# zhoujiahuan1991/ICCV2025-UPP

Hardware: AMD Instinct MI355X
Metric: point-clouds/sec fwd+bwd, UPP/Point-MAE N=1024 G=64 k=32 (higher is better)
Workload: dtype f32

## Files before the change

iccv2025-upp_amd/upp_hip/csrc/adapter.hip:

```cpp
#include "common.h"

namespace {

typedef float f32x16 __attribute__((ext_vector_type(16)));
constexpr int kH = 32;
constexpr int kRows = 32;
constexpr int kLG = 33;
constexpr int kAW = 8;
constexpr int kAT = 64 * kAW;

__device__ __forceinline__ int trow(int r, int lk) { return (r & 3) + 8 * (r >> 2) + 4 * lk; }
__device__ __forceinline__ void zero16(f32x16 &a) {
#pragma unroll
    for (int r = 0; r < 16; ++r) a[r] = 0.0f;
}
__device__ __forceinline__ float gelu_f(float x) { return 0.5f * x * (1.0f + erff(x * 0.70710678118654752440f)); }
__device__ __forceinline__ float gelu_grad(float x) {
    const float cdf = 0.5f * (1.0f + erff(x * 0.70710678118654752440f));
    const float pdf = 0.39894228040143267794f * expf(-0.5f * x * x);
    return cdf + x * pdf;
}

template <int NK, typename FA, typename FB>
__device__ __forceinline__ void mfma_chain(f32x16 &acc, FA fa, FB fb) {
// ... 308 lines not shown
#pragma unroll
    for (int t = 0; t < 2; ++t)
#pragma unroll
        for (int i = 0; i < NI; ++i)
            w1v[t][i] = *reinterpret_cast<const float4 *>(a.W1 + (size_t)(16 * t + r) * D + wave * KW + 16 * i + 4 * g);
#pragma unroll
    for (int t = 0; t < NT; ++t)
#pragma unroll
        for (int i = 0; i < 2; ++i)
            w2v[t][i] = *reinterpret_cast<const float4 *>(a.W2 + (size_t)(16 * (wave * NT + t) + r) * kH + 16 * i + 4 * g);

    {
        float gv[E], bv[E], ybv[E];
#pragma unroll
        for (int e = 0; e < E; ++e) {
            gv[e] = a.gamma[lane + 64 * e];
            bv[e] = a.beta[lane + 64 * e];
            ybv[e] = a.ybias ? a.ybias[lane + 64 * e] : 0.0f;
        }
        float xv[RW][E], yv[RW][E];
        int rowi[RW], bi[RW];
        [[maybe_unused]] int ci[RW];
        [[maybe_unused]] float pa[RW][E];
#pragma unroll
        for (int q = 0; q < RW; ++q) {
            const int row = min(row0 + wave * RW + q, R - 1);
            const int b = row / a.Lout, t = row - b * a.Lout;
            const int src = a.mode == 3 ? (t == 0 ? 0 : t + a.P) : (a.mode == 4 ? t + a.P : t);
            const size_t off = ((size_t)b * a.Lin + src) * D;
            rowi[q] = row; bi[q] = b;
            if constexpr (PROP) ci[q] = src - (a.Lin - a.T);
#pragma unroll
            for (int e = 0; e < E; ++e) {
                xv[q][e] = a.x[off + lane + 64 * e];
                yv[q][e] = a.y ? a.y[off + lane + 64 * e] : 0.0f;
            }
            for (int pp = 1; pp < a.yparts; ++pp) {
                float yp[E];
#pragma unroll
                for (int e = 0; e < E; ++e) yp[e] = a.y[(size_t)pp * a.ystride + off + lane + 64 * e];
#pragma unroll
                for (int e = 0; e < E; ++e) yv[q][e] += yp[e];
            }
        }
        if constexpr (PROP) {
            constexpr int kNb = 8, EC = 3;
            static_assert(E % EC == 0, "shape");
            float mu[E], rs[E], ga[E], be[E];
#pragma unroll
            for (int e = 0; e < E; ++e) {
                mu[e] = a.bn_mean[lane + 64 * e]; rs[e] = a.bn_rstd[lane + 64 * e];
                ga[e] = a.bn_gamma[lane + 64 * e]; be[e] = a.bn_beta[lane + 64 * e];
            }
#pragma unroll
            for (int q = 0; q < RW; ++q) {
                float acc[E];
#pragma unroll
                for (int e = 0; e < E; ++e) acc[e] = 0.0f;
                if (ci[q] >= 0) {
                    int j[kNb], cr[kNb];
                    float w[kNb], scr[kNb];
                    const size_t tok = ((size_t)bi[q] * a.T + ci[q]) * kNb;
#pragma unroll
                    for (int k = 0; k < kNb; ++k) { j[k] = a.idx8[tok + k]; w[k] = a.w8[tok + k]; }
#pragma unroll
                    for (int k = 0; k < kNb; ++k) cr[k] = a.i2[bi[q] * a.G2 + j[k]];
#pragma unroll
                    for (int k = 0; k < kNb; ++k) scr[k] = a.u ? floorf(a.keep + a.u[cr[k] / a.Lin]) / a.keep : 1.0f;
#pragma unroll
                    for (int h = 0; h < E; h += EC) {
                        float lv[EC][kNb], cx[EC][kNb], cy[EC][kNb];
#pragma unroll
                        for (int e = 0; e < EC; ++e)
#pragma unroll
                            for (int k = 0; k < kNb; ++k) {
                                const int c = lane + 64 * (h + e);
                                lv[e][k] = a.pooled[((size_t)bi[q] * a.G2 + j[k]) * D + c];
                                cx[e][k] = a.x[(size_t)cr[k] * D + c];
                                cy[e][k] = a.y[(size_t)cr[k] * D + c];
                            }
#pragma unroll
                        for (int e = 0; e < EC; ++e)
#pragma unroll
                            for (int k = 0; k < kNb; ++k) {
                                const float cv = __builtin_fmaf(cy[e][k] + ybv[h + e], scr[k], cx[e][k]);
                                const float lcv = ((lv[e][k] - mu[h + e]) * rs[h + e]) * ga[h + e] + be[h + e];
                                acc[h + e] += (lcv + 0.3f * cv) * w[k];
                            }
                    }
                }
#pragma unroll
                for (int e = 0; e < E; ++e) pa[q][e] = ci[q] >= 0 ? 0.3f * acc[e] : 0.0f;
            }
        }
#pragma unroll
        for (int q = 0; q < RW; ++q) {
            const int rr = wave * RW + q;
            const bool live = row0 + rr < R;
            const float sc = a.y ? (a.u ? floorf(a.keep + a.u[bi[q]]) / a.keep : 1.0f) : 0.0f;
            float v[E];
            float s = 0.0f;
#pragma unroll
            for (int e = 0; e < E; ++e) {
                float val = xv[q][e];
                if (a.y) val = __builtin_fmaf(yv[q][e] + ybv[e], sc, val);
                if constexpr (PROP) val = val + pa[q][e];
                v[e] = val;
                s += val;
            }
            const float mean = wave_sum_f32(s) / (float)D;
            float qq = 0.0f;
#pragma unroll
            for (int e = 0; e < E; ++e) { const float dv = v[e] - mean; qq = __builtin_fmaf(dv, dv, qq); }
            const float rstd = 1.0f / sqrtf(wave_sum_f32(qq) / (float)D + a.eps);
#pragma unroll
            for (int e = 0; e < E; ++e) {
                const float h = __builtin_fmaf((v[e] - mean) * rstd, gv[e], bv[e]);
                Hs[rr * LDH + lane + 64 * e] = live ? h : 0.0f;
                Vs[rr * LDH + lane + 64 * e] = v[e];
                if (live) a.xo[(size_t)rowi[q] * D + lane + 64 * e] = v[e];
            }
// ... 564 lines not shown
```

iccv2025-upp_amd/upp_hip/csrc/prop.hip:

```cpp
#include "common.h"

int upp_bn_finalize_launch(const float *part, int slabs, int per, int rows, int C, int training, float momentum, float eps,
                           float *running_mean, float *running_var, float *mean, float *rstd, hipStream_t st);

namespace {

constexpr int kMaxE = 8;
constexpr int kNb = 8;

__global__ __launch_bounds__(256) void prop_pool_fwd_kernel(const float *__restrict__ X, const int32_t *__restrict__ i1,
                                                            const float *__restrict__ u, float keep, float *__restrict__ pooled,
                                                            uint8_t *__restrict__ amax, int groups, int D) {
    const int lane = threadIdx.x & 63;
    const int g = blockIdx.x * 4 + __builtin_amdgcn_readfirstlane(threadIdx.x >> 6);
    if (g >= groups) return;
    const float f = 1.0f + (u ? floorf(keep + u[g]) / keep : 1.0f);
    float mx[kMaxE], sm[kMaxE];
    int am[kMaxE];
#pragma unroll
    for (int e = 0; e < kMaxE; ++e) { mx[e] = -__builtin_inff(); sm[e] = 0.0f; am[e] = 0; }
    int rows8[kNb];
#pragma unroll
    for (int k = 0; k < kNb; ++k) rows8[k] = i1[g * kNb + k];
    float val[kNb][kMaxE];
#pragma unroll
    for (int k = 0; k < kNb; ++k)
#pragma unroll
        for (int e = 0; e < kMaxE; ++e) val[k][e] = X[(size_t)rows8[k] * D + min(lane + 64 * e, D - 1)];
#pragma unroll
    for (int k = 0; k < kNb; ++k)
#pragma unroll
        for (int e = 0; e < kMaxE; ++e) {
            const float v = val[k][e] * f;
            if (v > mx[e]) { mx[e] = v; am[e] = k; }
            sm[e] += v;
        }
#pragma unroll
    for (int e = 0; e < kMaxE; ++e) {
        const int c = lane + 64 * e;
        if (c < D) { pooled[(size_t)g * D + c] = mx[e] + sm[e] * 0.125f; amax[(size_t)g * D + c] = (uint8_t)am[e]; }
    }
}

__device__ __forceinline__ int collect_hits(const int32_t *list, int n, int key, int *hits, int cap, int lane, int &q0) {
    int cnt = 0;
    int q = q0;
    for (; q < n && cnt + 64 <= cap; q += 64) {
        const int me = q + lane;
        const bool pred = me < n && list[me] == key;
        const unsigned long long mask = __ballot(pred);
        if (mask) {
            const int pos = cnt + __popcll(mask & ((1ull << lane) - 1ull));
            if (pred) hits[pos] = me;
            cnt += __popcll(mask);
        }
    }
    q0 = q;
    __builtin_amdgcn_wave_barrier();
    return cnt;
}
// ... 314 lines not shown
    }
}

__global__ __launch_bounds__(256) void prop_interp_bn_fwd_kernel(const float *__restrict__ X, const float *__restrict__ pooled,
                                                                 const float *__restrict__ mean, const float *__restrict__ rstd,
                                                                 const float *__restrict__ gamma, const float *__restrict__ beta,
                                                                 const int32_t *__restrict__ i2, const int32_t *__restrict__ idx8,
                                                                 const float *__restrict__ w8, float *__restrict__ out, int B, int Lp,
                                                                 int T, int G2, int D) {
    const int wgx = xcd_contiguous((int)blockIdx.x, (int)gridDim.x);
    const int lane = threadIdx.x & 63;
    const int r = wgx * 4 + __builtin_amdgcn_readfirstlane(threadIdx.x >> 6);
    if (r >= B * Lp) return;
    const int b = r / Lp, t = r - b * Lp;
    const int i = t - (Lp - T);
    int cc[kMaxE];
    float xv[kMaxE], acc[kMaxE];
#pragma unroll
    for (int e = 0; e < kMaxE; ++e) { cc[e] = min(lane + 64 * e, D - 1); xv[e] = X[(size_t)r * D + cc[e]]; acc[e] = 0.0f; }
    if (i >= 0) {
        int j[kNb], cr[kNb];
        float w[kNb];
#pragma unroll
        for (int k = 0; k < kNb; ++k) { j[k] = idx8[((size_t)b * T + i) * kNb + k]; w[k] = w8[((size_t)b * T + i) * kNb + k]; }
        float mu[kMaxE], rs[kMaxE], ga[kMaxE], be[kMaxE];
#pragma unroll
        for (int e = 0; e < kMaxE; ++e) { mu[e] = mean[cc[e]]; rs[e] = rstd[cc[e]]; ga[e] = gamma[cc[e]]; be[e] = beta[cc[e]]; }
#pragma unroll
        for (int k = 0; k < kNb; ++k) cr[k] = i2[b * G2 + j[k]];
#pragma unroll
        for (int h = 0; h < kMaxE; h += 4) {
            float lv[4][kNb], cv[4][kNb];
#pragma unroll
            for (int e = 0; e < 4; ++e)
#pragma unroll
                for (int k = 0; k < kNb; ++k) { lv[e][k] = pooled[((size_t)b * G2 + j[k]) * D + cc[h + e]]; cv[e][k] = X[(size_t)cr[k] * D + cc[h + e]]; }
#pragma unroll
            for (int e = 0; e < 4; ++e)
#pragma unroll
                for (int k = 0; k < kNb; ++k) {
                    const float lcv = ((lv[e][k] - mu[h + e]) * rs[h + e]) * ga[h + e] + be[h + e];
                    acc[h + e] += (lcv + 0.3f * cv[e][k]) * w[k];
                }
            if (64 * (h + 4) >= D) break;
        }
    }
#pragma unroll
    for (int e = 0; e < kMaxE; ++e) {
        const int c = lane + 64 * e;
        if (c < D) out[(size_t)r * D + c] = xv[e] + (i >= 0 ? 0.3f * acc[e] : 0.0f);
    }
}

__global__ __launch_bounds__(256) void prop_c2_csr_kernel(const float *__restrict__ g_out, const int32_t *__restrict__ start8,
                                                          const int32_t *__restrict__ perm8, const float *__restrict__ w8,
                                                          const float *__restrict__ pooled, const float *__restrict__ mean,
                                                          const float *__restrict__ rstd, float *__restrict__ g_c2,
                                                          float *__restrict__ part, int B, int Lp, int T, int G2, int D) {
    const int wgx = xcd_contiguous((int)blockIdx.x, (int)gridDim.x);
    __shared__ float sh[2][4][64 * kMaxE];
    const int lane = threadIdx.x & 63, wave = __builtin_amdgcn_readfirstlane(threadIdx.x >> 6);
    const int gj = wgx * 4 + wave;
    const int groups = B * G2;
    if (gj < groups) {
        int cc[kMaxE];
        float acc[kMaxE], pv[kMaxE], mu[kMaxE], rs[kMaxE];
#pragma unroll
        for (int e = 0; e < kMaxE; ++e) {
            cc[e] = min(lane + 64 * e, D - 1); acc[e] = 0.0f;
            pv[e] = pooled[(size_t)gj * D + cc[e]]; mu[e] = mean[cc[e]]; rs[e] = rstd[cc[e]];
        }
        const int s = start8[gj], eend = start8[gj + 1];
        for (int h0 = s; h0 < eend; h0 += 8) {
            int q[8];
#pragma unroll
            for (int t = 0; t < 8; ++t) q[t] = perm8[min(h0 + t, eend - 1)];
            float w[8];
            const float *grow[8];
#pragma unroll
            for (int t = 0; t < 8; ++t) {
                const int tok = q[t] / kNb;
                const int bb = tok / T, ii = tok - bb * T;
                w[t] = w8[q[t]];
                grow[t] = g_out + ((size_t)bb * Lp + (Lp - T) + ii) * D;
            }
            float gv[kMaxE][8];
#pragma unroll
            for (int e = 0; e < kMaxE; ++e)
#pragma unroll
                for (int t = 0; t < 8; ++t) gv[e][t] = grow[t][cc[e]];
#pragma unroll
            for (int t = 0; t < 8; ++t) {
                const float wt = h0 + t < eend ? w[t] : 0.0f;
#pragma unroll
                for (int e = 0; e < kMaxE; ++e) acc[e] += gv[e][t] * wt;
            }
        }
#pragma unroll
        for (int e = 0; e < kMaxE; ++e) {
            const int c = lane + 64 * e;
            if (c < D) {
                const float gl = 0.3f * acc[e];
                g_c2[(size_t)gj * D + c] = gl;
                sh[0][wave][c] = gl;
                sh[1][wave][c] = gl * ((pv[e] - mu[e]) * rs[e]);
            }
        }
    }
    __syncthreads();
    const int nw = min(4, groups - (int)wgx * 4);
    for (int c = threadIdx.x; c < D; c += 256) {
        float s0 = 0.0f, s1 = 0.0f;
        for (int w = 0; w < nw; ++w) { s0 += sh[0][w][c]; s1 += sh[1][w][c]; }
        part[((size_t)wgx * 2 + 0) * D + c] = s0;
        part[((size_t)wgx * 2 + 1) * D + c] = s1;
    }
}

__global__ __launch_bounds__(256) void prop_bn_grad_kernel(const float *__restrict__ part, int wgs, int D, float *__restrict__ g_gamma,
                                                           float *__restrict__ g_beta) {
    __shared__ float sb[4][64], sg[4][64];
    const int lane = threadIdx.x & 63, wave = threadIdx.x >> 6;
    const int c = blockIdx.x * 64 + lane;
    const int cc = min(c, D - 1);
    float ab = 0.0f, ag = 0.0f;
    for (int w0 = wave; w0 < wgs; w0 += 4 * 8) {
        float pb[8], pg[8];
#pragma unroll
        for (int t = 0; t < 8; ++t) {
            const int w = min(w0 + 4 * t, wgs - 1);
            pb[t] = part[((size_t)w * 2 + 0) * D + cc]; pg[t] = part[((size_t)w * 2 + 1) * D + cc];
        }
#pragma unroll
        for (int t = 0; t < 8; ++t) if (w0 + 4 * t < wgs) { ab += pb[t]; ag += pg[t]; }
    }
    sb[wave][lane] = ab; sg[wave][lane] = ag;
    __syncthreads();
    if (wave == 0 && c < D) {
        g_beta[c] = (sb[0][lane] + sb[1][lane]) + (sb[2][lane] + sb[3][lane]);
        g_gamma[c] = (sg[0][lane] + sg[1][lane]) + (sg[2][lane] + sg[3][lane]);
    }
}

__global__ __launch_bounds__(256) void prop_x_csr_kernel(const float *__restrict__ g_out, const float *__restrict__ g_c2,
                                                         const float *__restrict__ pooled, const uint8_t *__restrict__ amax,
                                                         const float *__restrict__ mean, const float *__restrict__ rstd,
                                                         const float *__restrict__ gamma, const float *__restrict__ g_gamma,
                                                         const float *__restrict__ g_beta, const float *__restrict__ u, float keep,
                                                         const int32_t *__restrict__ start1, const int32_t *__restrict__ perm1,
                                                         const int32_t *__restrict__ start2, const int32_t *__restrict__ perm2,
                                                         float *__restrict__ g_X, int rows, int groups, int D, int training) {
    const int wgx = xcd_contiguous((int)blockIdx.x, (int)gridDim.x);
    const int lane = threadIdx.x & 63;
    const int r = wgx * 4 + __builtin_amdgcn_readfirstlane(threadIdx.x >> 6);
    if (r >= rows) return;
    const int s1 = start1[r], e1 = start1[r + 1], s2 = start2[r], e2 = start2[r + 1];
    int cc[kMaxE];
    float acc[kMaxE], mu[kMaxE], rs[kMaxE], ga[kMaxE], c1[kMaxE], c2[kMaxE];
    const float inv_n = 1.0f / (float)groups;
#pragma unroll
    for (int e = 0; e < kMaxE; ++e) {
        cc[e] = min(lane + 64 * e, D - 1);
        acc[e] = g_out[(size_t)r * D + cc[e]];
        mu[e] = mean[cc[e]]; rs[e] = rstd[cc[e]]; ga[e] = gamma[cc[e]];
        c1[e] = 0.0f; c2[e] = 0.0f;
    }
    if (training) {
#pragma unroll
        for (int e = 0; e < kMaxE; ++e) { c1[e] = g_beta[cc[e]]; c2[e] = g_gamma[cc[e]]; }
    }
#pragma unroll
    for (int e = 0; e < kMaxE; ++e) { c1[e] *= inv_n; c2[e] *= inv_n; }
    for (int h0 = s2; h0 < e2; h0 += 2) {
        const int m0 = perm2[h0], m1 = perm2[min(h0 + 1, e2 - 1)];
        float a0[kMaxE], a1[kMaxE];
#pragma unroll
        for (int e = 0; e < kMaxE; ++e) { a0[e] = g_c2[(size_t)m0 * D + cc[e]]; a1[e] = g_c2[(size_t)m1 * D + cc[e]]; }
        const float f1 = h0 + 1 < e2 ? 0.3f : 0.0f;
#pragma unroll
        for (int e = 0; e < kMaxE; ++e) { acc[e] += 0.3f * a0[e]; acc[e] += f1 * a1[e]; }
    }
    auto add_entries = [&](int b0, int b1) {
        for (int h0 = b0; h0 < b1; h0 += 4) {
            int g[4], k[4];
            float f[4];
#pragma unroll
            for (int t = 0; t < 4; ++t) { const int q = perm1[min(h0 + t, b1 - 1)]; g[t] = q / kNb; k[t] = q - g[t] * kNb; }
#pragma unroll
            for (int t = 0; t < 4; ++t) f[t] = h0 + t < b1 ? 1.0f + (u ? floorf(keep + u[g[t]]) / keep : 1.0f) : 0.0f;
            float gl[kMaxE][4], pv[kMaxE][4];
            int am[kMaxE][4];
#pragma unroll
            for (int e = 0; e < kMaxE; ++e)
#pragma unroll
                for (int t = 0; t < 4; ++t) {
                    const size_t o = (size_t)g[t] * D + cc[e];
                    gl[e][t] = g_c2[o]; pv[e][t] = pooled[o]; am[e][t] = amax[o];
                }
#pragma unroll
            for (int e = 0; e < kMaxE; ++e)
#pragma unroll
                for (int t = 0; t < 4; ++t) {
                    const float xh = (pv[e][t] - mu[e]) * rs[e];
                    const float gp = (ga[e] * rs[e]) * (training ? gl[e][t] - c1[e] - xh * c2[e] : gl[e][t]);
                    acc[e] += gp * f[t] * (0.125f + (am[e][t] == k[t] ? 1.0f : 0.0f));
                }
        }
    };
    constexpr int kRowChunk = 64;
    if (e1 - s1 <= kRowChunk) {
        add_entries(s1, e1);
    } else {
        float head[kMaxE];
#pragma unroll
        for (int e = 0; e < kMaxE; ++e) head[e] = 0.0f;
        for (int c0 = s1; c0 < e1; c0 += kRowChunk) {
            if (c0 > s1) {
#pragma unroll
                for (int e = 0; e < kMaxE; ++e) { head[e] += acc[e]; acc[e] = 0.0f; }
            }
            add_entries(c0, min(e1, c0 + kRowChunk));
        }
#pragma unroll
        for (int e = 0; e < kMaxE; ++e) acc[e] += head[e];
    }
#pragma unroll
    for (int e = 0; e < kMaxE; ++e) { const int c = lane + 64 * e; if (c < D) g_X[(size_t)r * D + c] = acc[e]; }
}

__device__ __forceinline__ float res_scale(const float *u_dp, float keep_dp, int b) {
    return u_dp ? floorf(keep_dp + u_dp[b]) / keep_dp : 1.0f;
}

__global__ __launch_bounds__(256) void prop_pool_res_stats_kernel(const float *__restrict__ x2, const float *__restrict__ m,
                                                                  const float *__restrict__ mbias, const float *__restrict__ u_dp,
                                                                  float keep_dp, int Lp, const int32_t *__restrict__ i1,
                                                                  const float *__restrict__ u, float keep, float *__restrict__ pooled,
                                                                  uint8_t *__restrict__ amax, float *__restrict__ part, int groups, int D) {
    const int wgx = xcd_contiguous((int)blockIdx.x, (int)gridDim.x);
    __shared__ float sh[4][64 * kMaxE];
    const int lane = threadIdx.x & 63, wave = __builtin_amdgcn_readfirstlane(threadIdx.x >> 6);
    const int g = wgx * 4 + wave;
    if (g < groups) {
        const float f = 1.0f + (u ? floorf(keep + u[g]) / keep : 1.0f);
        int rows8[kNb];
        float sc[kNb];
#pragma unroll
        for (int k = 0; k < kNb; ++k) rows8[k] = i1[g * kNb + k];
#pragma unroll
        for (int k = 0; k < kNb; ++k) sc[k] = res_scale(u_dp, keep_dp, rows8[k] / Lp);
        float xv[kNb][kMaxE], mv[kNb][kMaxE], mb[kMaxE];
#pragma unroll
        for (int k = 0; k < kNb; ++k)
#pragma unroll
            for (int e = 0; e < kMaxE; ++e) {
                const size_t o = (size_t)rows8[k] * D + min(lane + 64 * e, D - 1);
                xv[k][e] = x2[o]; mv[k][e] = m[o];
            }
#pragma unroll
        for (int e = 0; e < kMaxE; ++e) mb[e] = mbias ? mbias[min(lane + 64 * e, D - 1)] : 0.0f;
#pragma unroll
        for (int e = 0; e < kMaxE; ++e) {
            float mx = -__builtin_inff(), sm = 0.0f;
            int am = 0;
#pragma unroll
            for (int k = 0; k < kNb; ++k) {
                const float v = __builtin_fmaf(mv[k][e] + mb[e], sc[k], xv[k][e]) * f;
                if (v > mx) { mx = v; am = k; }
                sm += v;
            }
            const int c = lane + 64 * e;
            const float pv = mx + sm * 0.125f;
            if (c < D) { pooled[(size_t)g * D + c] = pv; amax[(size_t)g * D + c] = (uint8_t)am; sh[wave][c] = pv; }
        }
    }
    __syncthreads();
    const int nw = min(4, groups - (int)wgx * 4);
    for (int c = threadIdx.x; c < D; c += 256) {
        float sum = 0.0f;
        for (int w = 0; w < nw; ++w) sum += sh[w][c];
        const float mean = sum / (float)nw;
        float m2 = 0.0f;
        for (int w = 0; w < nw; ++w) { const float dv = sh[w][c] - mean; m2 = __builtin_fmaf(dv, dv, m2); }
        part[((size_t)wgx * 2 + 0) * D + c] = sum;
        part[((size_t)wgx * 2 + 1) * D + c] = m2;
    }
}

__global__ __launch_bounds__(256) void prop_x_csr_res_kernel(const float *__restrict__ g_out, const float *__restrict__ g_c2,
                                                             const float *__restrict__ pooled, const uint8_t *__restrict__ amax,
                                                             const float *__restrict__ mean, const float *__restrict__ rstd,
                                                             const float *__restrict__ gamma, const float *__restrict__ g_gamma,
                                                             const float *__restrict__ g_beta, const float *__restrict__ u, float keep,
                                                             const int32_t *__restrict__ start1, const int32_t *__restrict__ perm1,
                                                             const int32_t *__restrict__ start2, const int32_t *__restrict__ perm2,
                                                             const float *__restrict__ u_dp, float keep_dp, int Lp,
                                                             float *__restrict__ g_x2, float *__restrict__ g_m, int rows, int groups, int D,
                                                             int training) {
    const int wgx = xcd_contiguous((int)blockIdx.x, (int)gridDim.x);
    const int lane = threadIdx.x & 63;
    const int r = wgx * 4 + __builtin_amdgcn_readfirstlane(threadIdx.x >> 6);
    if (r >= rows) return;
    const int s1 = start1[r], e1 = start1[r + 1], s2 = start2[r], e2 = start2[r + 1];
    const float sc = res_scale(u_dp, keep_dp, r / Lp);
    int cc[kMaxE];
    float acc[kMaxE], mu[kMaxE], rs[kMaxE], ga[kMaxE], c1[kMaxE], c2[kMaxE];
    const float inv_n = 1.0f / (float)groups;
#pragma unroll
    for (int e = 0; e < kMaxE; ++e) {
        cc[e] = min(lane + 64 * e, D - 1);
        acc[e] = g_out[(size_t)r * D + cc[e]];
        mu[e] = mean[cc[e]]; rs[e] = rstd[cc[e]]; ga[e] = gamma[cc[e]];
        c1[e] = 0.0f; c2[e] = 0.0f;
    }
    if (training) {
#pragma unroll
        for (int e = 0; e < kMaxE; ++e) { c1[e] = g_beta[cc[e]]; c2[e] = g_gamma[cc[e]]; }
    }
#pragma unroll
    for (int e = 0; e < kMaxE; ++e) { c1[e] *= inv_n; c2[e] *= inv_n; }
    for (int h0 = s2; h0 < e2; h0 += 2) {
        const int m0 = perm2[h0], m1 = perm2[min(h0 + 1, e2 - 1)];
        float a0[kMaxE], a1[kMaxE];
#pragma unroll
        for (int e = 0; e < kMaxE; ++e) { a0[e] = g_c2[(size_t)m0 * D + cc[e]]; a1[e] = g_c2[(size_t)m1 * D + cc[e]]; }
        const float f1 = h0 + 1 < e2 ? 0.3f : 0.0f;
#pragma unroll
        for (int e = 0; e < kMaxE; ++e) { acc[e] += 0.3f * a0[e]; acc[e] += f1 * a1[e]; }
    }
    auto add_entries = [&](int b0, int b1) {
        for (int h0 = b0; h0 < b1; h0 += 4) {
            int g[4], k[4];
            float f[4];
#pragma unroll
            for (int t = 0; t < 4; ++t) { const int q = perm1[min(h0 + t, b1 - 1)]; g[t] = q / kNb; k[t] = q - g[t] * kNb; }
#pragma unroll
            for (int t = 0; t < 4; ++t) f[t] = h0 + t < b1 ? 1.0f + (u ? floorf(keep + u[g[t]]) / keep : 1.0f) : 0.0f;
            float gl[kMaxE][4], pv[kMaxE][4];
            int am[kMaxE][4];
#pragma unroll
            for (int e = 0; e < kMaxE; ++e)
#pragma unroll
                for (int t = 0; t < 4; ++t) {
                    const size_t o = (size_t)g[t] * D + cc[e];
                    gl[e][t] = g_c2[o]; pv[e][t] = pooled[o]; am[e][t] = amax[o];
                }
#pragma unroll
            for (int e = 0; e < kMaxE; ++e)
#pragma unroll
                for (int t = 0; t < 4; ++t) {
                    const float xh = (pv[e][t] - mu[e]) * rs[e];
                    const float gp = (ga[e] * rs[e]) * (training ? gl[e][t] - c1[e] - xh * c2[e] : gl[e][t]);
                    acc[e] += gp * f[t] * (0.125f + (am[e][t] == k[t] ? 1.0f : 0.0f));
                }
        }
    };
    constexpr int kRowChunk = 64;
    if (e1 - s1 <= kRowChunk) {
        add_entries(s1, e1);
    } else {
        float head[kMaxE];
#pragma unroll
        for (int e = 0; e < kMaxE; ++e) head[e] = 0.0f;
        for (int c0 = s1; c0 < e1; c0 += kRowChunk) {
            if (c0 > s1) {
#pragma unroll
                for (int e = 0; e < kMaxE; ++e) { head[e] += acc[e]; acc[e] = 0.0f; }
            }
            add_entries(c0, min(e1, c0 + kRowChunk));
        }
#pragma unroll
        for (int e = 0; e < kMaxE; ++e) acc[e] += head[e];
    }
#pragma unroll
    for (int e = 0; e < kMaxE; ++e) {
        const int c = lane + 64 * e;
        if (c < D) { g_x2[(size_t)r * D + c] = acc[e]; g_m[(size_t)r * D + c] = acc[e] * sc; }
    }
}

__global__ __launch_bounds__(256) void prop_index_kernel(const float *__restrict__ c1, const float *__restrict__ c2,
                                                         const int64_t *__restrict__ i1, const int64_t *__restrict__ i2, int gather_idx,
                                                         int B, int T, int G2, int Lp, int off, float eps,
                                                         int32_t *__restrict__ i1a, int32_t *__restrict__ i2a,
                                                         int32_t *__restrict__ idx8, float *__restrict__ w8) {
    const int lane = threadIdx.x & 63;
    const int wg = blockIdx.x * 4 + __builtin_amdgcn_readfirstlane(threadIdx.x >> 6);
    {
        const int n1 = B * G2 * kNb, n2 = B * G2;
        const int e = wg * 64 + lane;
        if (e < n1 + n2) {
            const bool first = e < n1;
            const long long v = first ? i1[e] : i2[e - n1];
            long long r;
            if (gather_idx) {
                const int bsmp = first ? e / (G2 * kNb) : (e - n1) / G2;
                r = (long long)bsmp * Lp + off + v;
            } else {
                const int G = Lp - off;
                r = (v / G) * Lp + off + v % G;
            }
            if (first) i1a[e] = (int32_t)r; else i2a[e - n1] = (int32_t)r;
        }
    }
    if (wg >= B * T) return;
    const int b = wg / T;
    const float *a = c1 + (size_t)wg * 3;
    const float ax = a[0], ay = a[1], az = a[2];
    const int j = min(lane, G2 - 1);
    const float *q = c2 + ((size_t)b * G2 + j) * 3;
    const float bx = q[0], by = q[1], bz = q[2];
    float d = -2.0f * __builtin_fmaf(az, bz, __builtin_fmaf(ay, by, ax * bx));
    d += (ax * ax + ay * ay) + az * az;
    d += (bx * bx + by * by) + bz * bz;
    const uint32_t bits = __float_as_uint(d);
    uint32_t img = lane < G2 ? ((bits & 0x80000000u) ? ~bits : (bits | 0x80000000u)) : 0xFFFFFFFFu;
    float dk[kNb];
    int jk[kNb];
#pragma unroll
    for (int k = 0; k < kNb; ++k) {
        const uint32_t m = wave_min_u32(img);
        const int win = __builtin_ctzll(__ballot(img == m));
        jk[k] = win;
        dk[k] = __uint_as_float((m & 0x80000000u) ? (m & 0x7FFFFFFFu) : ~m);
        if (lane == win) img = 0xFFFFFFFFu;
    }
    float rc[kNb], sum = 0.0f;
#pragma unroll
    for (int k = 0; k < kNb; ++k) { rc[k] = 1.0f / (dk[k] + eps); sum += rc[k]; }
    if (lane < kNb) {
        float wv = 0.0f; int jv = 0;
// ... 167 lines not shown
    if (lds > 64 * 1024) return UPP_E_RANGE;
    const size_t lds_perm = lds + (size_t)2 * n * sizeof(int32_t);
    if (lds_perm <= 150 * 1024) {
        static std::atomic<bool> raised{false};
        if (!raised) {
            hipError_t e = hipFuncSetAttribute(reinterpret_cast<const void *>(csr_build_kernel<true>),
                                               hipFuncAttributeMaxDynamicSharedMemorySize, 150 * 1024);
            if (e != hipSuccess) return (int)e;
            raised = true;
        }
        hipLaunchKernelGGL(csr_build_kernel<true>, dim3(1), dim3(kCsrThreads), lds_perm, (hipStream_t)stream, keys, n, seg_len, seg_rows, rows,
                           start, perm);
    } else {
        hipLaunchKernelGGL(csr_build_kernel<false>, dim3(1), dim3(kCsrThreads), lds, (hipStream_t)stream, keys, n, seg_len, seg_rows, rows,
                           start, perm);
    }
    return upp_launch_status();
}

extern "C" long long upp_prop_part_floats(int groups, int D) {
    if (groups < 1 || D < 1) return 0;
    return (long long)((groups + 3) / 4) * 2 * D;
}

extern "C" int upp_prop_fwd(const float *X, const int32_t *i1, const float *u, float keep, const int32_t *i2, const int32_t *idx8,
                            const float *w8, const float *gamma, const float *beta, float *running_mean, float *running_var,
                            float momentum, float eps, int training, float *pooled, uint8_t *amax, float *part, float *mean,
                            float *rstd, float *out, int B, int Lp, int T, int G2, int D, void *stream) {
    if (!X || !i1 || !i2 || !idx8 || !w8 || !gamma || !beta || !pooled || !amax || !part || !mean || !rstd || !out) return UPP_E_BADARG;
    if (B < 1 || Lp < T || T < 1 || G2 < 1 || D < 1) return UPP_E_BADARG;
    if (!training && (!running_mean || !running_var)) return UPP_E_BADARG;
    if (D > 64 * kMaxE) return UPP_E_RANGE;
    hipStream_t st = (hipStream_t)stream;
    const int groups = B * G2, wgs = (groups + 3) / 4;
    hipLaunchKernelGGL(prop_pool_stats_kernel, dim3(wgs), dim3(256), 0, st, X, i1, u, keep, pooled, amax, part, groups, D);
    upp_bn_finalize_launch(part, wgs, 4, groups, D, training, momentum, eps, running_mean, running_var, mean, rstd, st);
    hipLaunchKernelGGL(prop_interp_bn_fwd_kernel, rows_grid((long long)B * Lp), dim3(256), 0, st, X, pooled, mean, rstd, gamma, beta, i2,
                       idx8, w8, out, B, Lp, T, G2, D);
    return upp_launch_status();
}

extern "C" int upp_prop_bwd(const float *g_out, const float *pooled, const uint8_t *amax, const float *mean, const float *rstd,
                            const float *gamma, const float *u, float keep, const float *w8, const int32_t *start1,
                            const int32_t *perm1, const int32_t *start2, const int32_t *perm2, const int32_t *start8,
                            const int32_t *perm8, int training, float *g_c2, float *part, float *g_gamma, float *g_beta, float *g_X,
                            int B, int Lp, int T, int G2, int D, void *stream) {
    if (!g_out || !pooled || !amax || !mean || !rstd || !gamma || !w8 || !start1 || !perm1 || !start2 || !perm2 || !start8 || !perm8 ||
        !g_c2 || !part || !g_gamma || !g_beta || !g_X)
        return UPP_E_BADARG;
    if (B < 1 || Lp < T || T < 1 || G2 < 1 || D < 1) return UPP_E_BADARG;
    if (D > 64 * kMaxE) return UPP_E_RANGE;
    hipStream_t st = (hipStream_t)stream;
    const int groups = B * G2, wgs = (groups + 3) / 4;
    hipLaunchKernelGGL(prop_c2_csr_kernel, dim3(wgs), dim3(256), 0, st, g_out, start8, perm8, w8, pooled, mean, rstd, g_c2, part, B, Lp, T,
                       G2, D);
    hipLaunchKernelGGL(prop_bn_grad_kernel, dim3((D + 63) / 64), dim3(256), 0, st, part, wgs, D, g_gamma, g_beta);
    hipLaunchKernelGGL(prop_x_csr_kernel, rows_grid((long long)B * Lp), dim3(256), 0, st, g_out, g_c2, pooled, amax, mean, rstd, gamma,
                       g_gamma, g_beta, u, keep, start1, perm1, start2, perm2, g_X, B * Lp, groups, D, training);
    return upp_launch_status();
}

extern "C" int upp_prop_res_pool_fwd(const float *x2, const float *m, const float *mbias, const float *u_dp, float keep_dp,
                                     const int32_t *i1, const float *u, float keep, float *running_mean, float *running_var,
                                     float momentum, float eps, int training, float *pooled, uint8_t *amax, float *part, float *mean,
                                     float *rstd, int B, int Lp, int G2, int D, void *stream) {
    if (!x2 || !m || !i1 || !pooled || !amax || !part || !mean || !rstd) return UPP_E_BADARG;
    if (B < 1 || Lp < 1 || G2 < 1 || D < 1 || !(keep_dp > 0.0f) || !(keep > 0.0f)) return UPP_E_BADARG;
    if (!training && (!running_mean || !running_var)) return UPP_E_BADARG;
    if (D > 64 * kMaxE) return UPP_E_RANGE;
    hipStream_t st = (hipStream_t)stream;
    const int groups = B * G2, wgs = (groups + 3) / 4;
    hipLaunchKernelGGL(prop_pool_res_stats_kernel, dim3(wgs), dim3(256), 0, st, x2, m, mbias, u_dp, keep_dp, Lp, i1, u, keep, pooled, amax,
                       part, groups, D);
    upp_bn_finalize_launch(part, wgs, 4, groups, D, training, momentum, eps, running_mean, running_var, mean, rstd, st);
    return upp_launch_status();
}

extern "C" int upp_prop_res_bwd(const float *g_out, const float *pooled, const uint8_t *amax, const float *mean, const float *rstd,
                                const float *gamma, const float *u, float keep, const float *w8, const int32_t *start1,
                                const int32_t *perm1, const int32_t *start2, const int32_t *perm2, const int32_t *start8,
                                const int32_t *perm8, int training, const float *u_dp, float keep_dp, float *g_c2, float *part,
                                float *g_gamma, float *g_beta, float *g_x2, float *g_m, int B, int Lp, int T, int G2, int D, void *stream) {
    if (!g_out || !pooled || !amax || !mean || !rstd || !gamma || !w8 || !start1 || !perm1 || !start2 || !perm2 || !start8 || !perm8 ||
        !g_c2 || !part || !g_gamma || !g_beta || !g_x2 || !g_m)
        return UPP_E_BADARG;
    if (B < 1 || Lp < T || T < 1 || G2 < 1 || D < 1 || !(keep_dp > 0.0f)) return UPP_E_BADARG;
    if (D > 64 * kMaxE) return UPP_E_RANGE;
    hipStream_t st = (hipStream_t)stream;
    const int groups = B * G2, wgs = (groups + 3) / 4;
    hipLaunchKernelGGL(prop_c2_csr_kernel, dim3(wgs), dim3(256), 0, st, g_out, start8, perm8, w8, pooled, mean, rstd, g_c2, part, B, Lp, T,
                       G2, D);
    hipLaunchKernelGGL(prop_bn_grad_kernel, dim3((D + 63) / 64), dim3(256), 0, st, part, wgs, D, g_gamma, g_beta);
    hipLaunchKernelGGL(prop_x_csr_res_kernel, rows_grid((long long)B * Lp), dim3(256), 0, st, g_out, g_c2, pooled, amax, mean, rstd, gamma,
                       g_gamma, g_beta, u, keep, start1, perm1, start2, perm2, u_dp, keep_dp, Lp, g_x2, g_m, B * Lp, groups, D, training);
    return upp_launch_status();
}

extern "C" int upp_prop_w8_grad(const float *g_out, const float *X, const float *pooled, const float *mean, const float *rstd,
                                const float *gamma, const float *beta, const int32_t *i2, const int32_t *idx8, float *g_w8, int B, int Lp,
                                int T, int G2, int D, void *stream) {
    if (!g_out || !X || !pooled || !i2 || !idx8 || !g_w8 || B < 1 || Lp < T || T < 1 || G2 < 1 || D < 1) return UPP_E_BADARG;
    if (mean && (!rstd || !gamma || !beta)) return UPP_E_BADARG;
    if (D > 64 * kMaxE) return UPP_E_RANGE;
    hipLaunchKernelGGL(prop_w8_grad_kernel, dim3((unsigned)(((long long)B * T + 3) / 4)), dim3(256), 0, (hipStream_t)stream, g_out, X, pooled,
                       mean, rstd, gamma, beta, i2, idx8, g_w8, B, Lp, T, G2, D);
    return upp_launch_status();
}

extern "C" int upp_prop_weights_bwd(const float *c1, const float *c2, const int32_t *idx8, const float *g_w8, float eps, float *g_c1,
                                    float *g_c2, int B, int T, int G2, void *stream) {
    if (!c1 || !c2 || !idx8 || !g_w8 || !g_c1 || !g_c2 || B < 1 || T < 1 || G2 < 1) return UPP_E_BADARG;
    const size_t lds = (size_t)T * kNb * (sizeof(float) + sizeof(int));
    if (lds > 64 * 1024) return UPP_E_RANGE;
    hipLaunchKernelGGL(prop_weights_bwd_kernel, dim3((unsigned)B), dim3(64), lds, (hipStream_t)stream, c1, c2, idx8, g_w8, eps, g_c1, g_c2, T, G2);
    return upp_launch_status();
}
```

Before: 7242.

## Cooperatively load CSR indices per wave and specialize prop kernels on channel width

In the adapter propagation path and in the prop backward CSR kernels, each lane now loads one index or weight from the CSR arrays and the values are passed around with readlane. Before, every lane issued redundant scalar-pattern loads per neighbour. The prop_c2 and prop_x CSR kernels become templates on the per-lane channel count E, so that D<=384 uses 6 instead of 8 slots and cuts registers and masked loads. The c2 gather is software-pipelined with double buffers, and the BN-grad reduction issues wider batches of loads. The two duplicated prop_x kernels are merged into one shared row function.

```diff
diff --git a/iccv2025-upp_amd/upp_hip/csrc/adapter.hip b/iccv2025-upp_amd/upp_hip/csrc/adapter.hip
--- a/iccv2025-upp_amd/upp_hip/csrc/adapter.hip
+++ b/iccv2025-upp_amd/upp_hip/csrc/adapter.hip
@@ -384,6 +384,15 @@
                 mu[e] = a.bn_mean[lane + 64 * e]; rs[e] = a.bn_rstd[lane + 64 * e];
                 ga[e] = a.bn_gamma[lane + 64 * e]; be[e] = a.bn_beta[lane + 64 * e];
             }
+            static_assert(RW * kNb <= 64, "shape");
+            int bl = bi[0], cl = ci[0];
+#pragma unroll
+            for (int q = 1; q < RW; ++q) if ((lane >> 3) == q) { bl = bi[q]; cl = ci[q]; }
+            const size_t tokl = ((size_t)bl * a.T + max(cl, 0)) * kNb + (lane & 7);
+            const int jl = a.idx8[tokl];
+            const float wl = a.w8[tokl];
+            const int crl = a.i2[bl * a.G2 + jl];
+            const float scl = a.u ? floorf(a.keep + a.u[crl / a.Lin]) / a.keep : 1.0f;
 #pragma unroll
             for (int q = 0; q < RW; ++q) {
                 float acc[E];
@@ -392,13 +401,13 @@
                 if (ci[q] >= 0) {
                     int j[kNb], cr[kNb];
                     float w[kNb], scr[kNb];
-                    const size_t tok = ((size_t)bi[q] * a.T + ci[q]) * kNb;
-#pragma unroll
-                    for (int k = 0; k < kNb; ++k) { j[k] = a.idx8[tok + k]; w[k] = a.w8[tok + k]; }
-#pragma unroll
-                    for (int k = 0; k < kNb; ++k) cr[k] = a.i2[bi[q] * a.G2 + j[k]];
-#pragma unroll
-                    for (int k = 0; k < kNb; ++k) scr[k] = a.u ? floorf(a.keep + a.u[cr[k] / a.Lin]) / a.keep : 1.0f;
+#pragma unroll
+                    for (int k = 0; k < kNb; ++k) {
+                        j[k] = __builtin_amdgcn_readlane(jl, kNb * q + k);
+                        cr[k] = __builtin_amdgcn_readlane(crl, kNb * q + k);
+                        w[k] = __int_as_float(__builtin_amdgcn_readlane(__float_as_int(wl), kNb * q + k));
+                        scr[k] = __int_as_float(__builtin_amdgcn_readlane(__float_as_int(scl), kNb * q + k));
+                    }
 #pragma unroll
                     for (int h = 0; h < E; h += EC) {
                         float lv[EC][kNb], cx[EC][kNb], cy[EC][kNb];
diff --git a/iccv2025-upp_amd/upp_hip/csrc/prop.hip b/iccv2025-upp_amd/upp_hip/csrc/prop.hip
--- a/iccv2025-upp_amd/upp_hip/csrc/prop.hip
+++ b/iccv2025-upp_amd/upp_hip/csrc/prop.hip
@@ -6,6 +6,11 @@
 namespace {
 
 constexpr int kMaxE = 8;
+#define PROP_LAUNCH_E(D, kernel, ...)                                          \
+    do {                                                                       \
+        if ((D) <= 64 * 6) hipLaunchKernelGGL(kernel<6>, __VA_ARGS__);         \
+        else hipLaunchKernelGGL(kernel<kMaxE>, __VA_ARGS__);                   \
+    } while (0)
 constexpr int kNb = 8;
 
 __global__ __launch_bounds__(256) void prop_pool_fwd_kernel(const float *__restrict__ X, const int32_t *__restrict__ i1,
@@ -426,52 +431,61 @@
     }
 }
 
+__device__ __forceinline__ int lane_get(int v, int l) { return __builtin_amdgcn_readlane(v, l); }
+__device__ __forceinline__ float lane_get(float v, int l) { return __int_as_float(__builtin_amdgcn_readlane(__float_as_int(v), l)); }
+constexpr int kSweep = 64;
+
+template <int E>
 __global__ __launch_bounds__(256) void prop_c2_csr_kernel(const float *__restrict__ g_out, const int32_t *__restrict__ start8,
                                                           const int32_t *__restrict__ perm8, const float *__restrict__ w8,
                                                           const float *__restrict__ pooled, const float *__restrict__ mean,
                                                           const float *__restrict__ rstd, float *__restrict__ g_c2,
                                                           float *__restrict__ part, int B, int Lp, int T, int G2, int D) {
     const int wgx = xcd_contiguous((int)blockIdx.x, (int)gridDim.x);
-    __shared__ float sh[2][4][64 * kMaxE];
+    __shared__ float sh[2][4][64 * E];
     const int lane = threadIdx.x & 63, wave = __builtin_amdgcn_readfirstlane(threadIdx.x >> 6);
     const int gj = wgx * 4 + wave;
     const int groups = B * G2;
     if (gj < groups) {
-        int cc[kMaxE];
-        float acc[kMaxE], pv[kMaxE], mu[kMaxE], rs[kMaxE];
-#pragma unroll
-        for (int e = 0; e < kMaxE; ++e) {
+        const int s = start8[gj], eend = start8[gj + 1];
+        int cc[E];
+        float acc[E], pv[E], mu[E], rs[E];
+#pragma unroll
+        for (int e = 0; e < E; ++e) {
             cc[e] = min(lane + 64 * e, D - 1); acc[e] = 0.0f;
             pv[e] = pooled[(size_t)gj * D + cc[e]]; mu[e] = mean[cc[e]]; rs[e] = rstd[cc[e]];
         }
-        const int s = start8[gj], eend = start8[gj + 1];
-        for (int h0 = s; h0 < eend; h0 += 8) {
-            int q[8];
-#pragma unroll
-            for (int t = 0; t < 8; ++t) q[t] = perm8[min(h0 + t, eend - 1)];
-            float w[8];
-            const float *grow[8];
-#pragma unroll
-            for (int t = 0; t < 8; ++t) {
-                const int tok = q[t] / kNb;
-                const int bb = tok / T, ii = tok - bb * T;
-                w[t] = w8[q[t]];
-                grow[t] = g_out + ((size_t)bb * Lp + (Lp - T) + ii) * D;
-            }
-            float gv[kMaxE][8];
-#pragma unroll
-            for (int e = 0; e < kMaxE; ++e)
-#pragma unroll
-                for (int t = 0; t < 8; ++t) gv[e][t] = grow[t][cc[e]];
-#pragma unroll
-            for (int t = 0; t < 8; ++t) {
-                const float wt = h0 + t < eend ? w[t] : 0.0f;
-#pragma unroll
-                for (int e = 0; e < kMaxE; ++e) acc[e] += gv[e][t] * wt;
-            }
-        }
-#pragma unroll
-        for (int e = 0; e < kMaxE; ++e) {
+        for (int c0 = s; c0 < eend; c0 += kSweep) {
+            const int q = perm8[min(c0 + lane, eend - 1)];
+            const float wq = w8[q];
+            const int tok = q / kNb;
+            const int bb = tok / T, ii = tok - bb * T;
+            const int rq = bb * Lp + (Lp - T) + ii;
+            const int nb = (min(kSweep, eend - c0) + 7) / 8;
+            auto load = [&](float (&gv)[E][8], int b) {
+#pragma unroll
+                for (int t = 0; t < 8; ++t) {
+                    const float *grow = g_out + (size_t)lane_get(rq, 8 * b + t) * D;
+#pragma unroll
+                    for (int e = 0; e < E; ++e) gv[e][t] = grow[cc[e]];
+                }
+            };
+            auto add = [&](const float (&gv)[E][8], int b) {
+#pragma unroll
+                for (int t = 0; t < 8; ++t) {
+                    const float wt = c0 + 8 * b + t < eend ? lane_get(wq, 8 * b + t) : 0.0f;
+#pragma unroll
+                    for (int e = 0; e < E; ++e) acc[e] += gv[e][t] * wt;
+                }
+            };
+            float ga[E][8], gb[E][8];
+            load(ga, 0);
+            int b = 0;
+            for (; b + 2 < nb; b += 2) { load(gb, b + 1); add(ga, b); load(ga, b + 2); add(gb, b + 1); }
+            if (b + 1 < nb) { load(gb, b + 1); add(ga, b); add(gb, b + 1); } else add(ga, b);
+        }
+#pragma unroll
+        for (int e = 0; e < E; ++e) {
             const int c = lane + 64 * e;
             if (c < D) {
                 const float gl = 0.3f * acc[e];
@@ -498,15 +512,19 @@
     const int c = blockIdx.x * 64 + lane;
     const int cc = min(c, D - 1);
     float ab = 0.0f, ag = 0.0f;
-    for (int w0 = wave; w0 < wgs; w0 += 4 * 8) {
-        float pb[8], pg[8];
-#pragma unroll
-        for (int t = 0; t < 8; ++t) {
-            const int w = min(w0 + 4 * t, wgs - 1);
-            pb[t] = part[((size_t)w * 2 + 0) * D + cc]; pg[t] = part[((size_t)w * 2 + 1) * D + cc];
-        }
-#pragma unroll
-        for (int t = 0; t < 8; ++t) if (w0 + 4 * t < wgs) { ab += pb[t]; ag += pg[t]; }
+    for (int w0 = wave; w0 < wgs; w0 += 4 * 64) {
+        float pb[2][32], pg[2][32];
+#pragma unroll
+        for (int h = 0; h < 2; ++h)
+#pragma unroll
+            for (int t = 0; t < 32; ++t) {
+                const int w = min(w0 + 4 * (32 * h + t), wgs - 1);
+                pb[h][t] = part[((size_t)w * 2 + 0) * D + cc]; pg[h][t] = part[((size_t)w * 2 + 1) * D + cc];
+            }
+#pragma unroll
+        for (int h = 0; h < 2; ++h)
+#pragma unroll
+            for (int t = 0; t < 32; ++t) if (w0 + 4 * (32 * h + t) < wgs) { ab += pb[h][t]; ag += pg[h][t]; }
     }
     sb[wave][lane] = ab; sg[wave][lane] = ag;
     __syncthreads();
@@ -516,6 +534,116 @@
     }
 }
 
+__device__ __forceinline__ float res_scale(const float *u_dp, float keep_dp, int b) {
+    return u_dp ? floorf(keep_dp + u_dp[b]) / keep_dp : 1.0f;
+}
+
+template <int E> struct XBatch { float gl[E][4], pv[E][4]; int am[E][4]; };
+
+template <int E, bool RES>
+__device__ __forceinline__ void prop_x_csr_row(const float *__restrict__ g_out, const float *__restrict__ g_c2,
+                                               const float *__restrict__ pooled, const uint8_t *__restrict__ amax,
+                                               const float *__restrict__ mean, const float *__restrict__ rstd,
+                                               const float *__restrict__ gamma, const float *__restrict__ g_gamma,
+                                               const float *__restrict__ g_beta, const float *__restrict__ u, float keep,
+                                               const int32_t *__restrict__ start1, const int32_t *__restrict__ perm1,
+                                               const int32_t *__restrict__ start2, const int32_t *__restrict__ perm2,
+                                               const float *__restrict__ u_dp, float keep_dp, int Lp, float *__restrict__ g_X,
+                                               float *__restrict__ g_m, int rows, int groups, int D, int training) {
+    const int wgx = xcd_contiguous((int)blockIdx.x, (int)gridDim.x);
+    const int lane = threadIdx.x & 63;
+    const int r = wgx * 4 + __builtin_amdgcn_readfirstlane(threadIdx.x >> 6);
+    if (r >= rows) return;
+    const int s1 = start1[r], e1 = start1[r + 1], s2 = start2[r], e2 = start2[r + 1];
+    constexpr int kRowChunk = kSweep;
+    int q = 0, m2 = 0;
+    if (e1 > s1) q = perm1[min(s1 + lane, min(e1, s1 + kRowChunk) - 1)];
+    if (e2 > s2) m2 = perm2[min(s2 + lane, e2 - 1)];
+    const float sc = RES ? res_scale(u_dp, keep_dp, r / Lp) : 1.0f;
+    int cc[E];
+    float acc[E], mu[E], rs[E], ga[E], c1[E], c2[E];
+    const float inv_n = 1.0f / (float)groups;
+#pragma unroll
+    for (int e = 0; e < E; ++e) {
+        cc[e] = min(lane + 64 * e, D - 1);
+        acc[e] = g_out[(size_t)r * D + cc[e]];
+        mu[e] = mean[cc[e]]; rs[e] = rstd[cc[e]]; ga[e] = gamma[cc[e]];
+        c1[e] = 0.0f; c2[e] = 0.0f;
+    }
+    if (training) {
+#pragma unroll
+        for (int e = 0; e < E; ++e) { c1[e] = g_beta[cc[e]]; c2[e] = g_gamma[cc[e]]; }
+    }
+#pragma unroll
+    for (int e = 0; e < E; ++e) { c1[e] *= inv_n; c2[e] *= inv_n; }
+    auto add_entries = [&](int b0, int b1, int qs) {
+        const int g = qs / kNb, k = qs - g * kNb;
+        const float f = 1.0f + (u ? floorf(keep + u[g]) / keep : 1.0f);
+        const int nb = (b1 - b0 + 3) / 4;
+        auto load = [&](XBatch<E> &x, int b) {
+#pragma unroll
+            for (int t = 0; t < 4; ++t) {
+                const size_t o = (size_t)lane_get(g, 4 * b + t) * D;
+#pragma unroll
+                for (int e = 0; e < E; ++e) { x.gl[e][t] = g_c2[o + cc[e]]; x.pv[e][t] = pooled[o + cc[e]]; x.am[e][t] = amax[o + cc[e]]; }
+            }
+        };
+        auto add = [&](const XBatch<E> &x, int b) {
+            float ft[4];
+            int kt[4];
+#pragma unroll
+            for (int t = 0; t < 4; ++t) { ft[t] = b0 + 4 * b + t < b1 ? lane_get(f, 4 * b + t) : 0.0f; kt[t] = lane_get(k, 4 * b + t); }
+#pragma unroll
+            for (int e = 0; e < E; ++e)
+#pragma unroll
+                for (int t = 0; t < 4; ++t) {
+                    const float xh = (x.pv[e][t] - mu[e]) * rs[e];
+                    const float gp = (ga[e] * rs[e]) * (training ? x.gl[e][t] - c1[e] - xh * c2[e] : x.gl[e][t]);
+                    acc[e] += gp * ft[t] * (0.125f + (x.am[e][t] == kt[t] ? 1.0f : 0.0f));
+                }
+        };
+        for (int b = 0; b < nb; ++b) { XBatch<E> x; load(x, b); add(x, b); }
+    };
+    for (int c0 = s2; c0 < e2; c0 += kSweep) {
+        if (c0 > s2) m2 = perm2[min(c0 + lane, e2 - 1)];
+        const int n = min(kSweep, e2 - c0);
+        for (int h = 0; h < n; h += 2) {
+            const size_t o0 = (size_t)lane_get(m2, h) * D, o1 = (size_t)lane_get(m2, h + 1) * D;
+            float a0[E], a1[E];
+#pragma unroll
+            for (int e = 0; e < E; ++e) { a0[e] = g_c2[o0 + cc[e]]; a1[e] = g_c2[o1 + cc[e]]; }
+            const float f1 = h + 1 < n ? 0.3f : 0.0f;
+#pragma unroll
+            for (int e = 0; e < E; ++e) { acc[e] += 0.3f * a0[e]; acc[e] += f1 * a1[e]; }
+        }
+    }
+    float head[E];
+#pragma unroll
+    for (int e = 0; e < E; ++e) head[e] = 0.0f;
+    for (int c0 = s1; c0 < e1; c0 += kRowChunk) {
+        const int b1 = min(e1, c0 + kRowChunk);
+        if (c0 > s1) {
+            q = perm1[min(c0 + lane, b1 - 1)];
+#pragma unroll
+            for (int e = 0; e < E; ++e) { head[e] += acc[e]; acc[e] = 0.0f; }
+        }
+        add_entries(c0, b1, q);
+    }
+    if (e1 - s1 > kRowChunk) {
+#pragma unroll
+        for (int e = 0; e < E; ++e) acc[e] += head[e];
+    }
+#pragma unroll
+    for (int e = 0; e < E; ++e) {
+        const int c = lane + 64 * e;
+        if (c < D) {
+            g_X[(size_t)r * D + c] = acc[e];
+            if (RES) g_m[(size_t)r * D + c] = acc[e] * sc;
+        }
+    }
+}
+
+template <int E>
 __global__ __launch_bounds__(256) void prop_x_csr_kernel(const float *__restrict__ g_out, const float *__restrict__ g_c2,
                                                          const float *__restrict__ pooled, const uint8_t *__restrict__ amax,
                                                          const float *__restrict__ mean, const float *__restrict__ rstd,
@@ -524,86 +652,8 @@
                                                          const int32_t *__restrict__ start1, const int32_t *__restrict__ perm1,
                                                          const int32_t *__restrict__ start2, const int32_t *__restrict__ perm2,
                                                          float *__restrict__ g_X, int rows, int groups, int D, int training) {
-    const int wgx = xcd_contiguous((int)blockIdx.x, (int)gridDim.x);
-    const int lane = threadIdx.x & 63;
-    const int r = wgx * 4 + __builtin_amdgcn_readfirstlane(threadIdx.x >> 6);
-    if (r >= rows) return;
-    const int s1 = start1[r], e1 = start1[r + 1], s2 = start2[r], e2 = start2[r + 1];
-    int cc[kMaxE];
-    float acc[kMaxE], mu[kMaxE], rs[kMaxE], ga[kMaxE], c1[kMaxE], c2[kMaxE];
-    const float inv_n = 1.0f / (float)groups;
-#pragma unroll
-    for (int e = 0; e < kMaxE; ++e) {
-        cc[e] = min(lane + 64 * e, D - 1);
-        acc[e] = g_out[(size_t)r * D + cc[e]];
-        mu[e] = mean[cc[e]]; rs[e] = rstd[cc[e]]; ga[e] = gamma[cc[e]];
-        c1[e] = 0.0f; c2[e] = 0.0f;
-    }
-    if (training) {
-#pragma unroll
-        for (int e = 0; e < kMaxE; ++e) { c1[e] = g_beta[cc[e]]; c2[e] = g_gamma[cc[e]]; }
-    }
-#pragma unroll
-    for (int e = 0; e < kMaxE; ++e) { c1[e] *= inv_n; c2[e] *= inv_n; }
-    for (int h0 = s2; h0 < e2; h0 += 2) {
-        const int m0 = perm2[h0], m1 = perm2[min(h0 + 1, e2 - 1)];
-        float a0[kMaxE], a1[kMaxE];
-#pragma unroll
-        for (int e = 0; e < kMaxE; ++e) { a0[e] = g_c2[(size_t)m0 * D + cc[e]]; a1[e] = g_c2[(size_t)m1 * D + cc[e]]; }
-        const float f1 = h0 + 1 < e2 ? 0.3f : 0.0f;
-#pragma unroll
-        for (int e = 0; e < kMaxE; ++e) { acc[e] += 0.3f * a0[e]; acc[e] += f1 * a1[e]; }
-    }
-    auto add_entries = [&](int b0, int b1) {
-        for (int h0 = b0; h0 < b1; h0 += 4) {
-            int g[4], k[4];
-            float f[4];
-#pragma unroll
-            for (int t = 0; t < 4; ++t) { const int q = perm1[min(h0 + t, b1 - 1)]; g[t] = q / kNb; k[t] = q - g[t] * kNb; }
-#pragma unroll
-            for (int t = 0; t < 4; ++t) f[t] = h0 + t < b1 ? 1.0f + (u ? floorf(keep + u[g[t]]) / keep : 1.0f) : 0.0f;
-            float gl[kMaxE][4], pv[kMaxE][4];
-            int am[kMaxE][4];
-#pragma unroll
-            for (int e = 0; e < kMaxE; ++e)
-#pragma unroll
-                for (int t = 0; t < 4; ++t) {
-                    const size_t o = (size_t)g[t] * D + cc[e];
-                    gl[e][t] = g_c2[o]; pv[e][t] = pooled[o]; am[e][t] = amax[o];
-                }
-#pragma unroll
-            for (int e = 0; e < kMaxE; ++e)
-#pragma unroll
-                for (int t = 0; t < 4; ++t) {
-                    const float xh = (pv[e][t] - mu[e]) * rs[e];
-                    const float gp = (ga[e] * rs[e]) * (training ? gl[e][t] - c1[e] - xh * c2[e] : gl[e][t]);
-                    acc[e] += gp * f[t] * (0.125f + (am[e][t] == k[t] ? 1.0f : 0.0f));
-                }
-        }
-    };
-    constexpr int kRowChunk = 64;
-    if (e1 - s1 <= kRowChunk) {
-        add_entries(s1, e1);
-    } else {
-        float head[kMaxE];
-#pragma unroll
-        for (int e = 0; e < kMaxE; ++e) head[e] = 0.0f;
-        for (int c0 = s1; c0 < e1; c0 += kRowChunk) {
-            if (c0 > s1) {
-#pragma unroll
-                for (int e = 0; e < kMaxE; ++e) { head[e] += acc[e]; acc[e] = 0.0f; }
-            }
-            add_entries(c0, min(e1, c0 + kRowChunk));
-        }
-#pragma unroll
-        for (int e = 0; e < kMaxE; ++e) acc[e] += head[e];
-    }
-#pragma unroll
-    for (int e = 0; e < kMaxE; ++e) { const int c = lane + 64 * e; if (c < D) g_X[(size_t)r * D + c] = acc[e]; }
-}
-
-__device__ __forceinline__ float res_scale(const float *u_dp, float keep_dp, int b) {
-    return u_dp ? floorf(keep_dp + u_dp[b]) / keep_dp : 1.0f;
+    prop_x_csr_row<E, false>(g_out, g_c2, pooled, amax, mean, rstd, gamma, g_gamma, g_beta, u, keep, start1, perm1, start2, perm2, nullptr, 1.0f, 1,
+                             g_X, nullptr, rows, groups, D, training);
 }
 
 __global__ __launch_bounds__(256) void prop_pool_res_stats_kernel(const float *__restrict__ x2, const float *__restrict__ m,
@@ -661,6 +711,7 @@
     }
 }
 
+template <int E>
 __global__ __launch_bounds__(256) void prop_x_csr_res_kernel(const float *__restrict__ g_out, const float *__restrict__ g_c2,
                                                              const float *__restrict__ pooled, const uint8_t *__restrict__ amax,
                                                              const float *__restrict__ mean, const float *__restrict__ rstd,
@@ -671,86 +722,8 @@
                                                              const float *__restrict__ u_dp, float keep_dp, int Lp,
                                                              float *__restrict__ g_x2, float *__restrict__ g_m, int rows, int groups, int D,
                                                              int training) {
-    const int wgx = xcd_contiguous((int)blockIdx.x, (int)gridDim.x);
-    const int lane = threadIdx.x & 63;
-    const int r = wgx * 4 + __builtin_amdgcn_readfirstlane(threadIdx.x >> 6);
-    if (r >= rows) return;
-    const int s1 = start1[r], e1 = start1[r + 1], s2 = start2[r], e2 = start2[r + 1];
-    const float sc = res_scale(u_dp, keep_dp, r / Lp);
-    int cc[kMaxE];
-    float acc[kMaxE], mu[kMaxE], rs[kMaxE], ga[kMaxE], c1[kMaxE], c2[kMaxE];
-    const float inv_n = 1.0f / (float)groups;
-#pragma unroll
-    for (int e = 0; e < kMaxE; ++e) {
-        cc[e] = min(lane + 64 * e, D - 1);
-        acc[e] = g_out[(size_t)r * D + cc[e]];
-        mu[e] = mean[cc[e]]; rs[e] = rstd[cc[e]]; ga[e] = gamma[cc[e]];
-        c1[e] = 0.0f; c2[e] = 0.0f;
-    }
-    if (training) {
-#pragma unroll
-        for (int e = 0; e < kMaxE; ++e) { c1[e] = g_beta[cc[e]]; c2[e] = g_gamma[cc[e]]; }
-    }
-#pragma unroll
-    for (int e = 0; e < kMaxE; ++e) { c1[e] *= inv_n; c2[e] *= inv_n; }
-    for (int h0 = s2; h0 < e2; h0 += 2) {
-        const int m0 = perm2[h0], m1 = perm2[min(h0 + 1, e2 - 1)];
-        float a0[kMaxE], a1[kMaxE];
-#pragma unroll
-        for (int e = 0; e < kMaxE; ++e) { a0[e] = g_c2[(size_t)m0 * D + cc[e]]; a1[e] = g_c2[(size_t)m1 * D + cc[e]]; }
-        const float f1 = h0 + 1 < e2 ? 0.3f : 0.0f;
-#pragma unroll
-        for (int e = 0; e < kMaxE; ++e) { acc[e] += 0.3f * a0[e]; acc[e] += f1 * a1[e]; }
-    }
-    auto add_entries = [&](int b0, int b1) {
-        for (int h0 = b0; h0 < b1; h0 += 4) {
-            int g[4], k[4];
-            float f[4];
-#pragma unroll
-            for (int t = 0; t < 4; ++t) { const int q = perm1[min(h0 + t, b1 - 1)]; g[t] = q / kNb; k[t] = q - g[t] * kNb; }
-#pragma unroll
-            for (int t = 0; t < 4; ++t) f[t] = h0 + t < b1 ? 1.0f + (u ? floorf(keep + u[g[t]]) / keep : 1.0f) : 0.0f;
-            float gl[kMaxE][4], pv[kMaxE][4];
-            int am[kMaxE][4];
-#pragma unroll
-            for (int e = 0; e < kMaxE; ++e)
-#pragma unroll
-                for (int t = 0; t < 4; ++t) {
-                    const size_t o = (size_t)g[t] * D + cc[e];
-                    gl[e][t] = g_c2[o]; pv[e][t] = pooled[o]; am[e][t] = amax[o];
-                }
-#pragma unroll
-            for (int e = 0; e < kMaxE; ++e)
-#pragma unroll
-                for (int t = 0; t < 4; ++t) {
-                    const float xh = (pv[e][t] - mu[e]) * rs[e];
-                    const float gp = (ga[e] * rs[e]) * (training ? gl[e][t] - c1[e] - xh * c2[e] : gl[e][t]);
-                    acc[e] += gp * f[t] * (0.125f + (am[e][t] == k[t] ? 1.0f : 0.0f));
-                }
-        }
-    };
-    constexpr int kRowChunk = 64;
-    if (e1 - s1 <= kRowChunk) {
-        add_entries(s1, e1);
-    } else {
-        float head[kMaxE];
-#pragma unroll
-        for (int e = 0; e < kMaxE; ++e) head[e] = 0.0f;
-        for (int c0 = s1; c0 < e1; c0 += kRowChunk) {
-            if (c0 > s1) {
-#pragma unroll
-                for (int e = 0; e < kMaxE; ++e) { head[e] += acc[e]; acc[e] = 0.0f; }
-            }
-            add_entries(c0, min(e1, c0 + kRowChunk));
-        }
-#pragma unroll
-        for (int e = 0; e < kMaxE; ++e) acc[e] += head[e];
-    }
-#pragma unroll
-    for (int e = 0; e < kMaxE; ++e) {
-        const int c = lane + 64 * e;
-        if (c < D) { g_x2[(size_t)r * D + c] = acc[e]; g_m[(size_t)r * D + c] = acc[e] * sc; }
-    }
+    prop_x_csr_row<E, true>(g_out, g_c2, pooled, amax, mean, rstd, gamma, g_gamma, g_beta, u, keep, start1, perm1, start2, perm2, u_dp, keep_dp, Lp,
+                            g_x2, g_m, rows, groups, D, training);
 }
 
 __global__ __launch_bounds__(256) void prop_index_kernel(const float *__restrict__ c1, const float *__restrict__ c2,
@@ -1024,10 +997,10 @@
     if (D > 64 * kMaxE) return UPP_E_RANGE;
     hipStream_t st = (hipStream_t)stream;
     const int groups = B * G2, wgs = (groups + 3) / 4;
-    hipLaunchKernelGGL(prop_c2_csr_kernel, dim3(wgs), dim3(256), 0, st, g_out, start8, perm8, w8, pooled, mean, rstd, g_c2, part, B, Lp, T,
+    PROP_LAUNCH_E(D, prop_c2_csr_kernel, dim3(wgs), dim3(256), 0, st, g_out, start8, perm8, w8, pooled, mean, rstd, g_c2, part, B, Lp, T,
                        G2, D);
     hipLaunchKernelGGL(prop_bn_grad_kernel, dim3((D + 63) / 64), dim3(256), 0, st, part, wgs, D, g_gamma, g_beta);
-    hipLaunchKernelGGL(prop_x_csr_kernel, rows_grid((long long)B * Lp), dim3(256), 0, st, g_out, g_c2, pooled, amax, mean, rstd, gamma,
+    PROP_LAUNCH_E(D, prop_x_csr_kernel, rows_grid((long long)B * Lp), dim3(256), 0, st, g_out, g_c2, pooled, amax, mean, rstd, gamma,
                        g_gamma, g_beta, u, keep, start1, perm1, start2, perm2, g_X, B * Lp, groups, D, training);
     return upp_launch_status();
 }
@@ -1060,10 +1033,10 @@
     if (D > 64 * kMaxE) return UPP_E_RANGE;
     hipStream_t st = (hipStream_t)stream;
     const int groups = B * G2, wgs = (groups + 3) / 4;
-    hipLaunchKernelGGL(prop_c2_csr_kernel, dim3(wgs), dim3(256), 0, st, g_out, start8, perm8, w8, pooled, mean, rstd, g_c2, part, B, Lp, T,
+    PROP_LAUNCH_E(D, prop_c2_csr_kernel, dim3(wgs), dim3(256), 0, st, g_out, start8, perm8, w8, pooled, mean, rstd, g_c2, part, B, Lp, T,
                        G2, D);
     hipLaunchKernelGGL(prop_bn_grad_kernel, dim3((D + 63) / 64), dim3(256), 0, st, part, wgs, D, g_gamma, g_beta);
-    hipLaunchKernelGGL(prop_x_csr_res_kernel, rows_grid((long long)B * Lp), dim3(256), 0, st, g_out, g_c2, pooled, amax, mean, rstd, gamma,
+    PROP_LAUNCH_E(D, prop_x_csr_res_kernel, rows_grid((long long)B * Lp), dim3(256), 0, st, g_out, g_c2, pooled, amax, mean, rstd, gamma,
                        g_gamma, g_beta, u, keep, start1, perm1, start2, perm2, u_dp, keep_dp, Lp, g_x2, g_m, B * Lp, groups, D, training);
     return upp_launch_status();
 }
```

After: 7332, median of 6. +1.2%, better.
